# XuZhang1211/PVPUFormer

Measured on AMD Instinct MI355X. Metric: 448x448 images/sec fwd+bwd, ViT-B VPUFormer, higher is better.
Workload: dtype bf16

## Files before the change

include/vpu_hip.h:

```cpp
#ifndef VPU_HIP_H
#define VPU_HIP_H
#include <stdint.h>

#ifdef __cplusplus
extern "C" {
#endif

#define VPU_BF16 0
#define VPU_F32 1

#define VPU_EPI_BIAS 1
#define VPU_EPI_PREACT 2
#define VPU_EPI_GELU 4
#define VPU_EPI_RELU 8
#define VPU_EPI_DGELU 16
#define VPU_EPI_DRELU 32
#define VPU_EPI_RESID 64
#define VPU_EPI_AFFINE 128
#define VPU_EPI_ACCUM 256
#define VPU_EPI_OUT_F32 512
#define VPU_EPI_SAVE_DGELU 1024
#define VPU_EPI_MULAUX 2048

typedef struct vpu_gemm_desc {
// ... 171 lines not shown
                             void* stream);
int vpu_pixel_shuffle2_gn_stats(const void* in, void* out, const float* bias, double* stats, int32_t B, int32_t h, int32_t w,
                                int32_t C, int32_t dtype, void* stream);
int vpu_groupnorm_apply(const void* x, const float* w, const float* b, void* y, float* mean, float* rstd, const double* stats,
                        int32_t B, int64_t HW, int32_t C, float eps, int32_t gelu, int32_t dtype, void* stream);
int vpu_pixel_unshuffle2_nblk(int32_t C);
int vpu_pixel_unshuffle2_sums(const void* in, void* out, float* part, int32_t B, int32_t h, int32_t w, int32_t C,
                              int32_t dtype, void* stream);
int vpu_groupnorm_nchunk(void);
int vpu_groupnorm_fwd(const void* x, const float* w, const float* b, void* y, float* mean, float* rstd, double* stats,
                      int32_t B, int64_t HW, int32_t C, float eps, int32_t gelu, int32_t dtype, void* stream);
int vpu_groupnorm_bwd(const void* dy, const void* x, const float* w, const float* b, const float* mean,
                      const float* rstd, void* dx, float* part, double* stats, int32_t B, int64_t HW, int32_t C,
                      int32_t gelu, int32_t dtype, void* stream);
int vpu_bilinear_cl_fwd(const void* in, int32_t ld_in, void* out, int32_t ld_out, int32_t B, int32_t h, int32_t w,
                        int32_t H, int32_t W, int32_t C, int32_t dtype, void* stream);
int vpu_bilinear_cl_bwd(const void* dout, int32_t ld_out, void* din, int32_t ld_in, int32_t B, int32_t h, int32_t w,
                        int32_t H, int32_t W, int32_t C, int32_t dtype, void* stream);
int vpu_upsum_relu(void* io, const void* const* z, const int32_t* h, const int32_t* w, int32_t n, int32_t B, int32_t H,
                   int32_t W, int32_t C, int32_t dtype, void* stream);
int vpu_head_grad_fused(const void* dfn, const void* y, const float* inv, const float* dout, const void* x, const float* w,
                        const float* mask, void* dx, float* part, float* part_b, int64_t rows, int64_t HW, int32_t C,
                        int32_t dtype, void* stream);
int vpu_gate_stats(const void* Q, const void* Kt, float* cg, int32_t* argq, float* sg, int32_t* argc, int32_t B,
                   int32_t nq, int32_t N, int32_t C, int32_t dtype, void* stream);
int vpu_gate_apply(const void* x, const float* cg, const float* sg, void* out, int32_t B, int32_t N, int32_t C,
                   int32_t dtype, void* stream);
int vpu_gate_bwd(const void* dout, const void* x, const float* cg, const int32_t* argq, const float* sg,
                 const int32_t* argc, void* dx, int32_t accum, void* dQ, void* dK, float* part, int32_t B, int32_t nq,
                 int32_t N, int32_t C, int32_t dtype, void* stream);
int vpu_gate_fwd_n(const void* const* Q, const void* const* K, const void* x, void* const* out, float* cg, int32_t* argq,
                   float* sg, int32_t* argc, int32_t n, int32_t B, int32_t nq, int32_t N, int32_t C, int32_t dtype, void* stream);
int vpu_gate_bwd_n(const void* const* dout, const void* x, const float* cg, const int32_t* argq, const float* sg,
                   const int32_t* argc, void* dx, int32_t accum, void* const* dQ, void* const* dK, float* part, int32_t n,
                   int32_t B, int32_t nq, int32_t N, int32_t C, int32_t dtype, void* stream);
int vpu_convseg_fwd(const void* x, const float* w, const float* bias, const float* mask, float* out, int64_t rows,
                    int64_t HW, int32_t C, int32_t dtype, void* stream);
int vpu_convseg_bwd_nblk(int64_t rows);
int vpu_convseg_bwd(const float* dout, const void* x, const float* w, const float* mask, void* dx, int32_t accum,
                    float* part, float* part_b, int64_t rows, int64_t HW, int32_t C, int32_t dtype, void* stream);

int vpu_upsample_ac_fwd(const float* in, float* out, int64_t planes, int32_t h, int32_t w, int32_t H, int32_t W,
                        void* stream);
int vpu_upsample_ac_bwd(const float* dout, float* din, int64_t planes, int32_t h, int32_t w, int32_t H, int32_t W,
                        void* stream);
int vpu_p2cl_fwd_bwd(const float* prob, const float* gt, const int32_t* slot_mask_idx, const float* override_masks,
// ... 28 lines not shown
```

pvpuformer_amd/_lib.py:

```python
import ctypes as C
import os

_HERE = os.path.dirname(os.path.abspath(__file__))
LIB_PATH = os.path.join(_HERE, os.environ.get("VPU_LIB_FILE") or
                        ("libvpu_hip_diag.so" if os.environ.get("VPU_LIB_DIAG", "0") == "1" else "libvpu_hip.so"))

BF16, F32 = 0, 1

EPI_BIAS, EPI_PREACT, EPI_GELU, EPI_RELU, EPI_DGELU, EPI_DRELU = 1, 2, 4, 8, 16, 32
EPI_RESID, EPI_AFFINE, EPI_ACCUM, EPI_OUT_F32 = 64, 128, 256, 512
EPI_SAVE_DGELU, EPI_MULAUX = 1024, 2048


class GemmDesc(C.Structure):
    _fields_ = [
        ("A", C.c_void_p), ("B", C.c_void_p), ("C", C.c_void_p), ("bias", C.c_void_p), ("resid", C.c_void_p),
        ("aux", C.c_void_p), ("preact", C.c_void_p),
        ("M", C.c_int32), ("N", C.c_int32), ("K", C.c_int32),
        ("lda", C.c_int32), ("ldb", C.c_int32), ("ldc", C.c_int32), ("ldr", C.c_int32), ("ldaux", C.c_int32),
        ("batch", C.c_int32), ("inner", C.c_int32),
        ("sAo", C.c_int64), ("sAi", C.c_int64), ("sBo", C.c_int64), ("sBi", C.c_int64),
        ("sCo", C.c_int64), ("sCi", C.c_int64), ("sRo", C.c_int64), ("sRi", C.c_int64),
        ("transA", C.c_int32), ("transB", C.c_int32), ("dtype", C.c_int32), ("flags", C.c_int32),
        ("resid_period", C.c_int32),
# ... 74 lines not shown
    "vpu_masked_argmax": [_P, _P, _P, _I, _I, _I, _P],
    "vpu_error_masks": [_P, _P, _P, _P, _I, _I, _P],
    "vpu_roi_resize_batched": [_P, _I, _P, _I, _I, _I, _I, _P],
    "vpu_roi_paste_batched": [_P, _I, _P, _I, _I, _F, _F, _I, _P],
    "vpu_click_keys_batched": [_P, _I, _P, _P, _P, _I, _I, _I, _P],
    "vpu_box_prompts_batched": [_P, _I, _P, _I, _I, _I, _F, _P, _P, _P, _P, _P, _I, _P, _P, _P],
    "vpu_disk_maps": [_P, _P, _P, _I, _I, _I, _I, _F, _P],
    "vpu_patch_im2col": [_P, _P, _P, _I, _I, _I, _I, _I, _I, _P],
    "vpu_patch_im2col_prenorm": [_P, _P, _P, _I, _I, _I, _I, _I, _I, _P],
    "vpu_patch_im2col_floor": [_P, _P, _P, _I, _I, _I, _I, _I, _I, _I, _P],
    "vpu_window_permute": [_P, _P, _I, _I, _I, _I, _I, _I, _P],
    "vpu_space_to_depth2_crop": [_P, _P, _I, _I, _I, _I, _I, _P],
    "vpu_pixel_shuffle2": [_P, _P, _P, _I, _I, _I, _I, _I, _I, _P],
    "vpu_pixel_shuffle2_gn_stats": [_P, _P, _P, _P, _I, _I, _I, _I, _I, _P],
    "vpu_groupnorm_apply": [_P, _P, _P, _P, _P, _P, _P, _I, _L, _I, _F, _I, _I, _P],
    "vpu_pixel_unshuffle2_nblk": [_I],
    "vpu_pixel_unshuffle2_sums": [_P, _P, _P, _I, _I, _I, _I, _I, _P],
    "vpu_groupnorm_nchunk": [],
    "vpu_groupnorm_fwd": [_P, _P, _P, _P, _P, _P, _P, _I, _L, _I, _F, _I, _I, _P],
    "vpu_groupnorm_bwd": [_P, _P, _P, _P, _P, _P, _P, _P, _P, _I, _L, _I, _I, _I, _P],
    "vpu_bilinear_cl_fwd": [_P, _I, _P, _I, _I, _I, _I, _I, _I, _I, _I, _P],
    "vpu_bilinear_cl_bwd": [_P, _I, _P, _I, _I, _I, _I, _I, _I, _I, _I, _P],
    "vpu_head_grad_fused": [_P, _P, _P, _P, _P, _P, _P, _P, _P, _P, _L, _L, _I, _I, _P],
    "vpu_upsum_relu": [_P, C.POINTER(C.c_void_p), C.POINTER(C.c_int32), C.POINTER(C.c_int32), _I, _I, _I, _I, _I, _I, _P],
    "vpu_gate_stats": [_P, _P, _P, _P, _P, _P, _I, _I, _I, _I, _I, _P],
    "vpu_gate_apply": [_P, _P, _P, _P, _I, _I, _I, _I, _P],
    "vpu_gate_bwd": [_P, _P, _P, _P, _P, _P, _P, _I, _P, _P, _P, _I, _I, _I, _I, _I, _P],
    "vpu_gate_fwd_n": [C.POINTER(C.c_void_p), C.POINTER(C.c_void_p), _P, C.POINTER(C.c_void_p), _P, _P, _P, _P, _I, _I, _I, _I, _I, _I, _P],
    "vpu_gate_bwd_n": [C.POINTER(C.c_void_p), _P, _P, _P, _P, _P, _P, _I, C.POINTER(C.c_void_p), C.POINTER(C.c_void_p), _P, _I, _I, _I,
                       _I, _I, _I, _P],
    "vpu_convseg_fwd": [_P, _P, _P, _P, _P, _L, _L, _I, _I, _P],
    "vpu_convseg_bwd_nblk": [_L],
    "vpu_convseg_bwd": [_P, _P, _P, _P, _P, _I, _P, _P, _L, _L, _I, _I, _P],
    "vpu_upsample_ac_fwd": [_P, _P, _L, _I, _I, _I, _I, _P],
    "vpu_upsample_ac_bwd": [_P, _P, _L, _I, _I, _I, _I, _P],
    "vpu_p2cl_fwd_bwd": [_P, _P, _P, _P, _P, _P, _F, _I, _I, _I, _I, _P],
    "vpu_p2cl_up_nband": [_I, _I],
    "vpu_p2cl_up_fwd_bwd": [_P, _P, _P, _P, _P, _P, _F, _I, _I, _I, _I, _I, _I, _P],
    "vpu_nfl_dice_scratch_doubles": [_I],
    "vpu_nfl_dice_fwd_bwd": [_P, _P, _P, _P, _P, _F, _F, _I, _L, _P],
    "vpu_loss_finalize": [_P, _P, _I, _I, C.c_double, _F, _F, _F, _F, _P, _P],
    "vpu_adam_step": [_P, _P, _P, _P, _P, _L, _F, _F, _F, _F, _F, _I, _F, _P],
    "vpu_adam_step_groups": [_P, _P, _P, _P, _P, _L, _P, _P, _P, _I, _F, _F, _F, _I, _I, _F, _P],
    "vpu_adam_step_hyper": [_P, _P, _P, _P, _P, _L, _P, _P, _P, _P, _I, _F, _F, _F, _F, _I, _P],
    "vpu_gemm_set_option": [C.c_char_p, _I],
    "vpu_gemm_get_option": [C.c_char_p, C.POINTER(C.c_int32)],
# ... 40 lines not shown
```

pvpuformer_amd/csrc/spatial.hip:

```cpp
#include <stdlib.h>
#include "vpu_common.h"
#include "interp_ac.h"
#include "../../include/vpu_hip.h"

#define DISPATCH_T(dtype, ...)                                   \
    if ((dtype) == VPU_BF16) { using T = bf16_t; __VA_ARGS__ }   \
    else if ((dtype) == VPU_F32) { using T = float; __VA_ARGS__ } \
    else { vpu_set_error("bad dtype"); return VPU_ERR_ARG; }
#define ST reinterpret_cast<hipStream_t>(stream)

namespace {

__constant__ float c_mean[3] = {0.485f, 0.456f, 0.406f};
__constant__ float c_std[3] = {0.229f, 0.224f, 0.225f};

template <typename T, bool NORM = true, bool VEC = true>
__global__ __launch_bounds__(256) void patch_im2col_kernel(const float* __restrict__ img4,
                                                           const float* __restrict__ disks, T* __restrict__ cols,
                                                           int B, int H, int W, int P, int wg) {
    const int gw = W / P, gh = H / P;
    const int K3 = 3 * P * P, K3P = (K3 + 7) / 8 * 8;
    const int Tn = gw * gh, KK = 2 * K3P, chunks = KK / 8;
    const int64_t total = (int64_t)B * Tn * chunks;
    const int nwx = gw / wg;
// ... 1296 lines not shown
            for (int j = 0; j < 8; ++j) {
                dwa[j] += d * xv[j] * mk[j];
                const float t = iv * (g[j] - yv[j] * sdot) + d * wv[j] * mk[j];
                o[j] = xv[j] > 0.f ? t : 0.f;
            }
            store8(dx + row * C + c8, o);
        }
    }
#pragma unroll
    for (int j = 0; j < 8; ++j)
        for (int o = lpr; o < 64; o <<= 1) dwa[j] += __shfl_xor(dwa[j], o, 64);
    dba = wave_sum(dba);
    if (sub == 0) {
#pragma unroll
        for (int j = 0; j < 8; ++j) red[wave][c8 + j] = dwa[j];
    }
    if (lane == 0) redb[wave] = dba;
    __syncthreads();
    for (int c = threadIdx.x; c < C; c += 256)
        part[(int64_t)blockIdx.x * C + c] = red[0][c] + red[1][c] + red[2][c] + red[3][c];
    if (threadIdx.x == 0) part_b[blockIdx.x] = redb[0] + redb[1] + redb[2] + redb[3];
}

__global__ __launch_bounds__(256) void upsample_ac_fwd_kernel(const float* __restrict__ in, float* __restrict__ out,
                                                              int64_t planes, int h, int w, int H, int W) {
    const float sh = ac_scale(h, H), sw = ac_scale(w, W);
    const int64_t total = planes * H * W;
    for (int64_t i = (int64_t)blockIdx.x * 256 + threadIdx.x; i < total; i += (int64_t)gridDim.x * 256) {
        const int X = (int)(i % W), Y = (int)((i / W) % H);
        const int64_t pl = i / ((int64_t)W * H);
        out[i] = ac_sample(in + pl * h * w, w, h, w, sh, sw, Y, X);
    }
}
__global__ __launch_bounds__(256) void upsample_ac_bwd_kernel(const float* __restrict__ dout, float* __restrict__ din,
                                                              int64_t planes, int h, int w, int H, int W) {
    const float sh = H > 1 ? (float)(h - 1) / (float)(H - 1) : 0.f;
    const float sw = W > 1 ? (float)(w - 1) / (float)(W - 1) : 0.f;
    const float fh = sh > 0.f ? 1.f / sh : 0.f, fw = sw > 0.f ? 1.f / sw : 0.f;
    const int64_t total = planes * h * w;
    const bool small = total < ((int64_t)1 << 31);
    for (int64_t i = (int64_t)blockIdx.x * 256 + threadIdx.x; i < total; i += (int64_t)gridDim.x * 256) {
        int x, y;
        int64_t pl;
        if (small) {
            const unsigned iu = (unsigned)i, q = iu / (unsigned)w;
            x = (int)(iu - q * (unsigned)w); y = (int)(q % (unsigned)h); pl = q / (unsigned)h;
// ... 351 lines not shown
        return vpu_check_launch("vpu_convseg_bwd");
    }
    DISPATCH_T(dtype, convseg_bwd_kernel<T><<<nblk, 256, 0, ST>>>(dout, (const T*)x, w, mask, (T*)dx, accum, part,
                                                                 part_b, rows, HW, C, nblk);)
    return vpu_check_launch("vpu_convseg_bwd");
}
extern "C" int vpu_head_grad_fused(const void* dfn, const void* y, const float* inv, const float* dout, const void* x,
                                   const float* w, const float* mask, void* dx, float* part, float* part_b, int64_t rows,
                                   int64_t HW, int32_t C, int32_t dtype, void* stream) {
    vpu_clear_stale_error();
    if (dtype != VPU_BF16 || !(C == 64 || C == 128 || C == 256 || C == 512) || !dfn || !y || !inv || !dout || !x || !w ||
        !dx || !part || !part_b || rows < 1 ||
        (reinterpret_cast<uintptr_t>(dfn) | reinterpret_cast<uintptr_t>(y) | reinterpret_cast<uintptr_t>(x) |
         reinterpret_cast<uintptr_t>(dx)) % 16 != 0 ||
        (reinterpret_cast<uintptr_t>(w) | reinterpret_cast<uintptr_t>(mask)) % 32 != 0) {
        vpu_set_error("head_grad_fused: bf16, C in {64,128,256,512}, 16-byte aligned maps, 32-byte aligned w / mask");
        return VPU_ERR_ARG;
    }
    const int nblk = vpu_convseg_bwd_nblk(rows);
    head_grad_fused_kernel<<<nblk, 256, 0, ST>>>((const bf16_t*)dfn, (const bf16_t*)y, inv, dout, (const bf16_t*)x, w, mask,
                                                 (bf16_t*)dx, part, part_b, rows, HW, C, nblk);
    return vpu_check_launch("vpu_head_grad_fused");
}
extern "C" int vpu_upsample_ac_fwd(const float* in, float* out, int64_t planes, int32_t h, int32_t w, int32_t H,
                                   int32_t W, void* stream) {
    vpu_clear_stale_error();
    upsample_ac_fwd_kernel<<<vpu_grid_for(planes * H * W, 256, 65536), 256, 0, ST>>>(in, out, planes, h, w, H, W);
    return vpu_check_launch("vpu_upsample_ac_fwd");
}
extern "C" int vpu_upsample_ac_bwd(const float* dout, float* din, int64_t planes, int32_t h, int32_t w, int32_t H,
                                   int32_t W, void* stream) {
    vpu_clear_stale_error();
    upsample_ac_bwd_kernel<<<vpu_grid_for(planes * h * w, 256, 65536), 256, 0, ST>>>(dout, din, planes, h, w, H, W);
    return vpu_check_launch("vpu_upsample_ac_bwd");
}
```

pvpuformer_amd/engine.py:

```python
import contextlib
import math
import os
from collections import OrderedDict
from types import SimpleNamespace

import numpy as np
import torch

from . import ops
from ._lib import (BF16, F32, EPI_BIAS, EPI_PREACT, EPI_GELU, EPI_RELU, EPI_DGELU, EPI_DRELU, EPI_RESID, EPI_AFFINE,
                   EPI_ACCUM, EPI_OUT_F32, EPI_SAVE_DGELU, EPI_MULAUX)


class Tape:
    __slots__ = ("fns", "out_grads", "done", "sim_low", "lane")

    def __init__(self):
        self.fns = []
        self.out_grads = [None, None, None]
        self.done = False
        self.sim_low = None
        self.lane = None

    def append(self, fn):
# ... 89 lines not shown
        self.shadow_valid = False
        self._const_ready = False
        self.use_flash = True
        self.use_side = os.environ.get("VPU_WGRAD_STREAM", "0") == "1"
        self.side = None
        self.fuse_ln_pe = True
        self.group_wgrad = True
        self.ride_wgrad = True
        self.wgrad_fill = 0.8
        hid = self.D * c["mlp_ratio"]
        blk = sum(((n + 255) // 256) * ((k + 127) // 128) for n, k in ((3 * self.D, self.D), (self.D, self.D), (hid, self.D), (self.D, hid)))
        pk = os.environ.get("VPU_WGRAD_PACK", "")
        k3 = ops.gemm_get_option("k3")
        k4_default = (k3 & 8) != 0
        self.pack_wgrad = pk == "1" or (pk != "0" and (blk < 0.95 * 256 or k4_default))
        self.k3_wgrad = (k3 & 1) != 0
        self.k4_wgrad = (k3 & 8) != 0
        self.wgrad_round = 256 if (self.k4_wgrad or not self.k3_wgrad) else 512
        self.wgrad_tn = 256 if self.k4_wgrad else 128
        self.unify_wgrad = True
        self.lazy_zero = True
        self.xattn_split = max(1, int(os.environ.get("VPU_XATTN_SPLIT", "1")))
        self.neck_lanes = int(os.environ.get("VPU_NECK_LANES", "0"))
        self._tok_stream = None
        self._in_lanes = False
        self.dist_colsum = True
        self._pack_seen, self._pack_total = {}, {}
        self._pending_reports, self._reporting = [], False
        self.group_tiles = 256
        self.split_wgrad = True
        self._wq = []
        self._csq = []
        self._gq = []
        self._gq_out = set()
        self._frozen = set()
        self._token_rows = 0
        self.grad_ready_hook = None
        self.report_lag = max(1, int(os.environ.get("VPU_DIST_REPORT_LAG", "2")))

    def bind(self, named_params):
        self.names = OrderedDict()
        off = 0
        for n, p in named_params.items():
            self.names[n] = (off, tuple(p.shape), p.numel())
            off = _rup(off + p.numel(), 8)
        self.total = off
# ... 975 lines not shown
        if cx.training:
            def bwd_fusion():
                if fused.g is None:
                    return
                if relu_done[0]:
                    dt_ = fused.g
                else:
                    dt_ = self._new(B * HW4, Cc)
                    ops.act_bwd(fused.g, Cc, fused.t, Cc, dt_, Cc, B * HW4, Cc, 0, self.dt)
                self._wgrad(dt_, Cc, ys[0].t, Cc, gf, Cc, Cc, B * HW4, ldc=ldf, bias="head.fusion_conv.conv.bias")
                fuse_mask = self.dt == BF16
                mk = dict(flags=EPI_DRELU, ldaux=Cc) if fuse_mask else {}
                self._dgrad(dt_, Cc, wf, ldf, ys[0], B * HW4, Cc, Cc, **(dict(mk, aux=ys[0].t) if fuse_mask else {}))
                ymask[0][0] = fuse_mask
                for i in (1, 2, 3):
                    s = feats[i][1]
                    dz = self._new(B * s * s, Cc)
                    ops.bilinear_cl_bwd(dt_, Cc, dz, Cc, B, s, s, Hs, Hs, Cc, self.dt)
                    self._wgrad(dz, Cc, ys[i].t, Cc, (gf[0], gf[1] + i * Cc), Cc, Cc, B * s * s, ldc=ldf)
                    self._dgrad(dz, Cc, (wf[0], wf[1] + i * Cc), ldf, ys[i], B * s * s, Cc, Cc,
                                **(dict(mk, aux=ys[i].t) if fuse_mask else {}))
                    ymask[i][0] = fuse_mask
            self.tape.append(bwd_fusion)
        seg = self._new(B * HW4, dtype=torch.float32)
        ops.convseg_fwd(fused.t, self.Pm("head.conv_seg.weight"), self.Pm("head.conv_seg.bias"), drop_mask, seg,
                        B * HW4, HW4, Cc)
        dm = self.cfg["head_d_model"]
        query = self.mlp(q_out, "head.ffn_layer.lin1", "head.ffn_layer.lin2", B * nq, dm, 2 * dm, Cc, "relu")
        qn, fn = Var(torch.empty_like(query.t)), Var(torch.empty_like(fused.t))
        inv_q, inv_f = self._new(B * nq, dtype=torch.float32), self._new(B * HW4, dtype=torch.float32)
        ops.l2norm_fwd(query.t, qn.t, inv_q, B * nq, Cc)
        ops.l2norm_fwd(fused.t, fn.t, inv_f, B * HW4, Cc)
        sim = self._new(B, nq, HW4, dtype=torch.float32)
        ops.gemm(qn.t, fn.t, sim, nq, HW4, Cc, Cc, Cc, HW4, self.dt, flags=EPI_OUT_F32 | EPI_AFFINE, post_mul=0.5,
                 post_add=0.5, batch=B, inner=1, sA=(nq * Cc, 0), sB=(HW4 * Cc, 0), sC=(nq * HW4, 0))
        if cx.taps is not None:
            cx.taps["seg_lowres"] = seg.view(B, 1, Hs, Hs)
            cx.taps["sim_lowres"] = sim.view(B, nq, Hs, Hs)
            cx.taps["fused"] = fused.t
        inst = self._new(B, 1, H, W_, dtype=torch.float32)
        ops.upsample_ac_fwd(seg, inst, B, Hs, Hs, H, W_)
        aux = None
        self.sim_low = sim.view(B, nq, Hs, Hs)
        if materialize_aux:
            aux = self._new(B, nq, H, W_, dtype=torch.float32)
            ops.upsample_ac_fwd(sim, aux, B * nq, Hs, Hs, H, W_)
        tape.sim_low = self.sim_low
        if cx.training:
            def bwd_head():
                d_inst, d_aux, d_sim_low = tape.out_grads
                if d_aux is not None or d_sim_low is not None:
                    if d_sim_low is not None:
                        dsim = d_sim_low.view(B, nq, HW4)
                    else:
                        dsim = self._new(B, nq, HW4, dtype=torch.float32)
                        ops.upsample_ac_bwd(d_aux, dsim, B * nq, Hs, Hs, H, W_)
                    if self.dt == BF16:
                        dsim_t = self._new(B, nq, HW4)
                        ops.cast2d(dsim, HW4, dsim_t, HW4, B * nq, HW4)
                    else:
                        dsim_t = dsim
                    qn.g, fn.g = torch.empty_like(qn.t), torch.empty_like(fn.t)
                    ops.gemm(dsim_t, fn.t, qn.g, nq, Cc, HW4, HW4, Cc, Cc, self.dt, transB=True, alpha=0.5, batch=B,
                             inner=1, sA=(nq * HW4, 0), sB=(HW4 * Cc, 0), sC=(nq * Cc, 0))
                    ops.gemm(dsim_t, qn.t, fn.g, HW4, Cc, nq, HW4, Cc, Cc, self.dt, transA=True, transB=True, alpha=0.5,
                             batch=B, inner=1, sA=(nq * HW4, 0), sB=(nq * Cc, 0), sC=(HW4 * Cc, 0))
                    query.g = torch.empty_like(query.t)
                    ops.l2norm_bwd(qn.g, qn.t, inv_q, query.g, B * nq, Cc)
                    one_pass = d_inst is not None and self.dt == BF16 and Cc in (64, 128, 256, 512)
                    if not one_pass:
                        fused.g = torch.empty_like(fused.t)
                        ops.l2norm_bwd(fn.g, fn.t, inv_f, fused.g, B * HW4, Cc)
                if d_inst is not None:
# ... 306 lines not shown
```

pvpuformer_amd/ops.py:

```python
import ctypes as C

import torch

from . import _lib
from ._lib import (BF16, F32, EPI_BIAS, EPI_PREACT, EPI_GELU, EPI_RELU, EPI_DGELU, EPI_DRELU, EPI_RESID, EPI_AFFINE,
                   EPI_ACCUM, EPI_OUT_F32, EPI_SAVE_DGELU, EPI_MULAUX, GemmDesc)

TORCH_DTYPE = {BF16: torch.bfloat16, F32: torch.float32}


def code_of(t):
    if isinstance(t, tuple):
        t = t[0]
    if t.dtype == torch.bfloat16:
        return BF16
    if t.dtype == torch.float32:
        return F32
    raise TypeError(f"unsupported dtype {t.dtype}")


_raw_stream = getattr(torch._C, "_cuda_getCurrentRawStream", None)
_cur_device = getattr(torch._C, "_cuda_getDevice", None)


# ... 492 lines not shown
def gate_bwd_n(douts, x, cg, argq, sg, argc, dx, accum, dQs, dKs, part, B, nq, N, Cdim):
    _lib.call("vpu_gate_bwd_n", _ptr_array(douts), ptr(x), ptr(cg), ptr(argq), ptr(sg), ptr(argc), ptr(dx), int(accum),
              _ptr_array(dQs), _ptr_array(dKs), ptr(part), len(douts), B, nq, N, Cdim, code_of(x), _stream())


def convseg_fwd(x, w, bias, mask, out, rows, HW, Cdim):
    _lib.call("vpu_convseg_fwd", ptr(x), ptr(w), ptr(bias), ptr(mask), ptr(out), rows, HW, Cdim, code_of(x), _stream())


def convseg_bwd_nblk(rows):
    return _lib.load().vpu_convseg_bwd_nblk(rows)


def convseg_bwd(dout, x, w, mask, dx, accum, part, part_b, rows, HW, Cdim):
    _lib.call("vpu_convseg_bwd", ptr(dout), ptr(x), ptr(w), ptr(mask), ptr(dx), int(accum), ptr(part), ptr(part_b),
              rows, HW, Cdim, code_of(x), _stream())


def head_grad_fused(dfn, y, inv, dout, x, w, mask, dx, part, part_b, rows, HW, Cdim):
    _lib.call("vpu_head_grad_fused", ptr(dfn), ptr(y), ptr(inv), ptr(dout), ptr(x), ptr(w), ptr(mask), ptr(dx), ptr(part),
              ptr(part_b), rows, HW, Cdim, code_of(x), _stream())


def upsample_ac_fwd(inp, out, planes, h, w, H, W):
    _lib.call("vpu_upsample_ac_fwd", ptr(inp), ptr(out), planes, h, w, H, W, _stream())


def upsample_ac_bwd(dout, din, planes, h, w, H, W):
    _lib.call("vpu_upsample_ac_bwd", ptr(dout), ptr(din), planes, h, w, H, W, _stream())


def p2cl_fwd_bwd(prob, gt, slot_idx, override, loss_part, dprob, grad_scale, B, S, H, W):
    _lib.call("vpu_p2cl_fwd_bwd", ptr(prob), ptr(gt), ptr(slot_idx), ptr(override), ptr(loss_part), ptr(dprob),
              grad_scale, B, S, H, W, _stream())


def p2cl_up_fwd_bwd(sim_low, gt, slot_idx, override, loss_part, dsim_low, grad_scale, B, S, h, w, H, W):
    nband = _lib.load().vpu_p2cl_up_nband(h, w)
    bands = torch.empty(B * S, nband, device=sim_low.device, dtype=torch.float32)
    _lib.call("vpu_p2cl_up_fwd_bwd", ptr(sim_low), ptr(gt), ptr(slot_idx), ptr(override), ptr(bands), ptr(dsim_low),
              grad_scale, B, S, h, w, H, W, _stream())
    if loss_part is None:
        return bands
    torch.sum(bands, dim=1, out=loss_part.view(B * S))
    return loss_part

# ... 27 lines not shown
```

Before: 998.8.

## Fuse head conv_seg, feature L2 norm and similarity GEMM into row kernels

Adds fused forward and backward kernels for the segmentation head. The forward kernel computes the per-pixel inverse norm, the conv_seg dot product and the query-feature similarity with MFMA in a single pass over the fused features, so the normalized feature map is never written out. The backward kernel computes dx, including the L2-norm backward, conv_seg grad and ReLU mask, together with per-block partial query gradients. Separate small kernels reduce the query-gradient partials and the weight sums. This removes several full passes over the large feature map and a separate GEMM launch, at the cost of considerable new kernel complexity, and it applies only to bf16 with restricted C and nq.

```diff
diff --git a/include/vpu_hip.h b/include/vpu_hip.h
--- a/include/vpu_hip.h
+++ b/include/vpu_hip.h
@@ -217,6 +217,13 @@
 int vpu_head_grad_fused(const void* dfn, const void* y, const float* inv, const float* dout, const void* x, const float* w,
                         const float* mask, void* dx, float* part, float* part_b, int64_t rows, int64_t HW, int32_t C,
                         int32_t dtype, void* stream);
+int vpu_head_rows_fwd(const void* x, const void* qn, const float* w, const float* bias, const float* mask, float* seg,
+                      float* inv, float* sim, int32_t B, int64_t HW, int32_t nq, int32_t C, int32_t dtype, void* stream);
+int vpu_head_rows_bwd_nblk(int32_t B, int64_t HW, int32_t C);
+int vpu_head_rows_bwd(const void* x, const float* inv, const void* qn, const float* inv_q, const float* dsim,
+                      const float* dseg, const float* w, const float* mask, void* dx, float* part, float* part_b,
+                      float* dqn_part, void* dquery, int32_t B, int64_t HW, int32_t nq, int32_t C, int32_t dtype,
+                      void* stream);
 int vpu_gate_stats(const void* Q, const void* Kt, float* cg, int32_t* argq, float* sg, int32_t* argc, int32_t B,
                    int32_t nq, int32_t N, int32_t C, int32_t dtype, void* stream);
 int vpu_gate_apply(const void* x, const float* cg, const float* sg, void* out, int32_t B, int32_t N, int32_t C,
diff --git a/pvpuformer_amd/_lib.py b/pvpuformer_amd/_lib.py
--- a/pvpuformer_amd/_lib.py
+++ b/pvpuformer_amd/_lib.py
@@ -120,6 +120,9 @@
     "vpu_bilinear_cl_fwd": [_P, _I, _P, _I, _I, _I, _I, _I, _I, _I, _I, _P],
     "vpu_bilinear_cl_bwd": [_P, _I, _P, _I, _I, _I, _I, _I, _I, _I, _I, _P],
     "vpu_head_grad_fused": [_P, _P, _P, _P, _P, _P, _P, _P, _P, _P, _L, _L, _I, _I, _P],
+    "vpu_head_rows_fwd": [_P, _P, _P, _P, _P, _P, _P, _P, _I, _L, _I, _I, _I, _P],
+    "vpu_head_rows_bwd_nblk": [_I, _L, _I],
+    "vpu_head_rows_bwd": [_P, _P, _P, _P, _P, _P, _P, _P, _P, _P, _P, _P, _P, _I, _L, _I, _I, _I, _P],
     "vpu_upsum_relu": [_P, C.POINTER(C.c_void_p), C.POINTER(C.c_int32), C.POINTER(C.c_int32), _I, _I, _I, _I, _I, _I, _P],
     "vpu_gate_stats": [_P, _P, _P, _P, _P, _P, _I, _I, _I, _I, _I, _P],
     "vpu_gate_apply": [_P, _P, _P, _P, _I, _I, _I, _I, _P],
diff --git a/pvpuformer_amd/csrc/spatial.hip b/pvpuformer_amd/csrc/spatial.hip
--- a/pvpuformer_amd/csrc/spatial.hip
+++ b/pvpuformer_amd/csrc/spatial.hip
@@ -1342,6 +1342,363 @@
     if (threadIdx.x == 0) part_b[blockIdx.x] = redb[0] + redb[1] + redb[2] + redb[3];
 }
 
+typedef __bf16 bf16x4_t __attribute__((ext_vector_type(4)));
+__device__ __forceinline__ void hr_unpack(const uint4& u, float (&v)[8]) {
+    const bf16x8_t e = __builtin_bit_cast(bf16x8_t, u);
+#pragma unroll
+    for (int j = 0; j < 8; ++j) v[j] = (float)e[j];
+}
+__device__ __forceinline__ bf16x8_t hr_frag(const char* img, int row, int ld, int k) {
+    return *reinterpret_cast<const bf16x8_t*>(img + row * ld + k * 2);
+}
+constexpr int HR_LDP = 64 * 2 + 16;
+
+template <int C>
+__global__ __launch_bounds__(256) void head_rows_fwd_kernel(const bf16_t* __restrict__ x, const bf16_t* __restrict__ qn,
+                                                            const float* __restrict__ w, const float* __restrict__ bias,
+                                                            const float* __restrict__ mask, float* __restrict__ seg,
+                                                            float* __restrict__ inv, float* __restrict__ sim, int HW, int nq,
+                                                            int ntiles) {
+    extern __shared__ __attribute__((aligned(16))) char hr_lds[];
+    constexpr int LPR = C / 8, RPW = 64 / LPR, TRIPS = 16 / RPW, LD = C * 2 + 16;
+    char* sQ = hr_lds;
+    char* sF = sQ + nq * LD;
+    float* sS = reinterpret_cast<float*>(sF + 64 * LD);
+    const int tid = threadIdx.x, lane = tid & 63, wave = tid >> 6, sub = lane / LPR, cl = lane - sub * LPR;
+    const int b = blockIdx.y;
+    for (int i = tid; i < nq * LPR; i += 256) {
+        const int q = i / LPR, c8 = (i - q * LPR) * 8;
+        *reinterpret_cast<uint4*>(sQ + q * LD + c8 * 2) = *reinterpret_cast<const uint4*>(qn + ((int64_t)b * nq + q) * C + c8);
+    }
+    float ww[8], wm[8];
+    load8(w + cl * 8, ww);
+    if (mask) {
+        float mk[8];
+        load8(mask + (int64_t)b * C + cl * 8, mk);
+#pragma unroll
+        for (int j = 0; j < 8; ++j) wm[j] = ww[j] * mk[j];
+    } else {
+#pragma unroll
+        for (int j = 0; j < 8; ++j) wm[j] = ww[j];
+    }
+    const float b0 = bias[0];
+    const bf16_t* xb = x + (int64_t)b * HW * C;
+    const int prow = wave * 16 + sub;
+    uint4 raw[TRIPS];
+    int tile = blockIdx.x;
+    if (tile < ntiles) {
+#pragma unroll
+        for (int t = 0; t < TRIPS; ++t) {
+            const int hw = tile * 64 + prow + t * RPW;
+            raw[t] = make_uint4(0, 0, 0, 0);
+            if (hw < HW) raw[t] = *reinterpret_cast<const uint4*>(xb + (int64_t)hw * C + cl * 8);
+        }
+    }
+    for (; tile < ntiles; tile += gridDim.x) {
+        const int hw0 = tile * 64;
+#pragma unroll
+        for (int t = 0; t < TRIPS; ++t) {
+            const int p = prow + t * RPW, hw = hw0 + p;
+            float v[8];
+            hr_unpack(raw[t], v);
+            float s = 0.f, sg = 0.f;
+#pragma unroll
+            for (int j = 0; j < 8; ++j) s += v[j] * v[j];
+#pragma unroll
+            for (int j = 0; j < 8; ++j) sg += v[j] * wm[j];
+            for (int o = LPR >> 1; o > 0; o >>= 1) s += __shfl_xor(s, o, 64);
+            for (int o = LPR >> 1; o > 0; o >>= 1) sg += __shfl_xor(sg, o, 64);
+            const float iv = 1.0f / fmaxf(sqrtf(s), 1e-12f);
+            if (cl == 0 && hw < HW) {
+                inv[(int64_t)b * HW + hw] = iv;
+                seg[(int64_t)b * HW + hw] = sg + b0;
+            }
+            bf16x8_t f;
+#pragma unroll
+            for (int j = 0; j < 8; ++j) f[j] = (bf16_t)(v[j] * iv);
+            *reinterpret_cast<bf16x8_t*>(sF + p * LD + cl * 16) = f;
+        }
+        const int next = tile + gridDim.x;
+        if (next < ntiles) {
+#pragma unroll
+            for (int t = 0; t < TRIPS; ++t) {
+                const int hw = next * 64 + prow + t * RPW;
+                raw[t] = make_uint4(0, 0, 0, 0);
+                if (hw < HW) raw[t] = *reinterpret_cast<const uint4*>(xb + (int64_t)hw * C + cl * 8);
+            }
+        }
+        __syncthreads();
+        bf16x8_t fb[C / 32];
+#pragma unroll
+        for (int ks = 0; ks < C / 32; ++ks) fb[ks] = hr_frag(sF, wave * 16 + (lane & 15), LD, ks * 32 + 8 * (lane >> 4));
+        for (int mt = 0; mt < (nq >> 4); ++mt) {
+            f32x4_t acc = (f32x4_t){0.f, 0.f, 0.f, 0.f};
+#pragma unroll
+            for (int ks = 0; ks < C / 32; ++ks)
+                acc = __builtin_amdgcn_mfma_f32_16x16x32_bf16(hr_frag(sQ, mt * 16 + (lane & 15), LD, ks * 32 + 8 * (lane >> 4)),
+                                                              fb[ks], acc, 0, 0, 0);
+#pragma unroll
+            for (int r = 0; r < 4; ++r) sS[(mt * 16 + 4 * (lane >> 4) + r) * 64 + wave * 16 + (lane & 15)] = acc[r] * 0.5f + 0.5f;
+        }
+        __syncthreads();
+        if (hw0 + lane < HW)
+            for (int q = wave; q < nq; q += 4) sim[((int64_t)b * nq + q) * HW + hw0 + lane] = sS[q * 64 + lane];
+    }
+}
+
+template <int C>
+__global__ __launch_bounds__(256) void head_rows_bwd_kernel(const bf16_t* __restrict__ x, const float* __restrict__ inv,
+                                                            const bf16_t* __restrict__ qn, const float* __restrict__ dsim,
+                                                            const float* __restrict__ dseg, const float* __restrict__ w,
+                                                            const float* __restrict__ mask, bf16_t* __restrict__ dx,
+                                                            float* __restrict__ dqp, int HW, int nq, int ntiles_all, int G, int tpc) {
+    extern __shared__ __attribute__((aligned(16))) char hr_lds[];
+    constexpr int LPR = C / 8, RPW = 64 / LPR, TRIPS = 16 / RPW, LD = C * 2 + 16, NCT = C / 64;
+    const int KQ = (nq + 31) & ~31, LDQ = KQ * 2 + 16, nqt = nq >> 4, nks = KQ >> 5;
+    char* sQT = hr_lds;
+    char* sDT = sQT + C * LDQ;
+    char* sD = sDT + 64 * LDQ;
+    char* sGY = sD + 64 * HR_LDP;
+    const int tid = threadIdx.x, lane = tid & 63, wave = tid >> 6, sub = lane / LPR, cl = lane - sub * LPR, c8 = cl * 8;
+    const int b = blockIdx.x / G, g0 = blockIdx.x - b * G;
+    for (int i = tid; i < C * LDQ / 16; i += 256) reinterpret_cast<uint4*>(sQT)[i] = make_uint4(0, 0, 0, 0);
+    __syncthreads();
+    for (int i = tid; i < nq * LPR; i += 256) {
+        const int q = i / LPR, cc = (i - q * LPR) * 8;
+        const bf16x8_t e = *reinterpret_cast<const bf16x8_t*>(qn + ((int64_t)b * nq + q) * C + cc);
+#pragma unroll
+        for (int j = 0; j < 8; ++j) *reinterpret_cast<bf16_t*>(sQT + (cc + j) * LDQ + q * 2) = e[j];
+    }
+    float wv[8], mk[8] = {1.f, 1.f, 1.f, 1.f, 1.f, 1.f, 1.f, 1.f};
+    load8(w + c8, wv);
+    if (mask) load8(mask + (int64_t)b * C + c8, mk);
+    f32x4_t dq[4][NCT];
+#pragma unroll
+    for (int mt = 0; mt < 4; ++mt)
+#pragma unroll
+        for (int ct = 0; ct < NCT; ++ct) dq[mt][ct] = (f32x4_t){0.f, 0.f, 0.f, 0.f};
+    const int64_t rowb = (int64_t)b * HW;
+    const bf16_t* xb = x + rowb * C;
+    const float* dsb = dsim + (int64_t)b * nq * HW;
+    const int prow = wave * 16 + sub;
+    const int sp = tid & 63, sqg = tid >> 6;
+    constexpr bool PF = C <= 256;
+    uint4 raw[TRIPS], nraw[PF ? TRIPS : 1];
+    float ivr[TRIPS], dr[TRIPS], nivr[PF ? TRIPS : 1], ndr[PF ? TRIPS : 1], dsv[2][8], ndsv[2][8];
+#define HR_ISSUE(TILE_, RAW_, IV_, D_, DS_)                                                                            \
+    {                                                                                                                  \
+        _Pragma("unroll") for (int t = 0; t < TRIPS; ++t) {                                                            \
+            const int hw = (TILE_) * 64 + prow + t * RPW;                                                              \
+            RAW_[t] = make_uint4(0, 0, 0, 0);                                                                          \
+            IV_[t] = 0.f;                                                                                              \
+            D_[t] = 0.f;                                                                                               \
+            if (hw < HW) {                                                                                             \
+                RAW_[t] = *reinterpret_cast<const uint4*>(xb + (int64_t)hw * C + c8);                                  \
+                IV_[t] = inv[rowb + hw];                                                                               \
+                D_[t] = dseg[rowb + hw];                                                                               \
+            }                                                                                                          \
+        }                                                                                                              \
+        _Pragma("unroll") for (int u = 0; u < 2; ++u) _Pragma("unroll") for (int j = 0; j < 8; ++j) {                  \
+            const int q = (sqg + 4 * u) * 8 + j, hw = (TILE_) * 64 + sp;                                               \
+            DS_[u][j] = (q < nq && hw < HW) ? dsb[(int64_t)q * HW + hw] : 0.f;                                         \
+        }                                                                                                              \
+    }
+    int tile = g0 * tpc;
+    const int ntiles = (g0 + 1) * tpc < ntiles_all ? (g0 + 1) * tpc : ntiles_all;
+    if (tile < ntiles) HR_ISSUE(tile, raw, ivr, dr, dsv)
+    for (; tile < ntiles; ++tile) {
+        const int hw0 = tile * 64;
+#pragma unroll
+        for (int u = 0; u < 2; ++u) {
+            const int qg = sqg + 4 * u;
+            if (qg * 8 < KQ) {
+                bf16x8_t e;
+#pragma unroll
+                for (int j = 0; j < 8; ++j) e[j] = (bf16_t)dsv[u][j];
+                *reinterpret_cast<bf16x8_t*>(sDT + sp * LDQ + qg * 16) = e;
+                if (qg * 8 < nq) {
+#pragma unroll
+                    for (int j = 0; j < 8; ++j) *reinterpret_cast<bf16_t*>(sD + (qg * 8 + j) * HR_LDP + sp * 2) = e[j];
+                }
+            }
+        }
+#pragma unroll
+        for (int t = 0; t < TRIPS; ++t) {
+            float v[8];
+            hr_unpack(raw[t], v);
+            bf16x8_t f;
+#pragma unroll
+            for (int j = 0; j < 8; ++j) f[j] = (bf16_t)(v[j] * ivr[t]);
+            *reinterpret_cast<bf16x8_t*>(sGY + (prow + t * RPW) * LD + cl * 16) = f;
+        }
+        __syncthreads();
+        const int next = tile + 1;
+        if constexpr (PF) { if (next < ntiles) HR_ISSUE(next, nraw, nivr, ndr, ndsv) }
+#pragma unroll 1
+        for (int ks = 0; ks < 2; ++ks) {
+            bf16x8_t fa[4];
+#pragma unroll
+            for (int mt = 0; mt < 4; ++mt)
+                if (mt < nqt) fa[mt] = hr_frag(sD, mt * 16 + (lane & 15), HR_LDP, ks * 32 + 8 * (lane >> 4));
+#pragma unroll
+            for (int ct = 0; ct < NCT; ++ct) {
+                const int c = wave * (C / 4) + ct * 16 + (lane & 15);
+                bf16x8_t fb;
+#pragma unroll
+                for (int j = 0; j < 8; ++j)
+                    fb[j] = *reinterpret_cast<const bf16_t*>(sGY + (ks * 32 + 8 * (lane >> 4) + j) * LD + c * 2);
+#pragma unroll
+                for (int mt = 0; mt < 4; ++mt)
+                    if (mt < nqt) dq[mt][ct] = __builtin_amdgcn_mfma_f32_16x16x32_bf16(fa[mt], fb, dq[mt][ct], 0, 0, 0);
+            }
+        }
+        __syncthreads();
+        {
+            bf16x8_t fd[2];
+#pragma unroll
+            for (int ks = 0; ks < 2; ++ks)
+                if (ks < nks) fd[ks] = hr_frag(sDT, wave * 16 + (lane & 15), LDQ, ks * 32 + 8 * (lane >> 4));
+#pragma unroll 2
+            for (int ct = 0; ct < C / 16; ++ct) {
+                f32x4_t acc = (f32x4_t){0.f, 0.f, 0.f, 0.f};
+#pragma unroll
+                for (int ks = 0; ks < 2; ++ks)
+                    if (ks < nks)
+                        acc = __builtin_amdgcn_mfma_f32_16x16x32_bf16(
+                            hr_frag(sQT, ct * 16 + (lane & 15), LDQ, ks * 32 + 8 * (lane >> 4)), fd[ks], acc, 0, 0, 0);
+                bf16x4_t e;
+#pragma unroll
+                for (int r = 0; r < 4; ++r) e[r] = (bf16_t)(acc[r] * 0.5f);
+                *reinterpret_cast<bf16x4_t*>(sGY + (wave * 16 + (lane & 15)) * LD + (ct * 16 + 4 * (lane >> 4)) * 2) = e;
+            }
+        }
+        __syncthreads();
+#pragma unroll
+        for (int t = 0; t < TRIPS; ++t) {
+            const int p = prow + t * RPW, hw = hw0 + p;
+            const bool live = hw < HW;
+            float xv[8], gv[8], yv[8];
+            hr_unpack(raw[t], xv);
+            hr_unpack(*reinterpret_cast<const uint4*>(sGY + p * LD + cl * 16), gv);
+            const float iv = ivr[t], d = dr[t];
+#pragma unroll
+            for (int j = 0; j < 8; ++j) yv[j] = (float)(bf16_t)(xv[j] * iv);
+            float sdot = 0.f;
+#pragma unroll
+            for (int j = 0; j < 8; ++j) sdot += gv[j] * yv[j];
+            for (int o = LPR >> 1; o > 0; o >>= 1) sdot += __shfl_xor(sdot, o, 64);
+            if (live) {
+                float o[8];
+#pragma unroll
+                for (int j = 0; j < 8; ++j) {
+                    const float tt = iv * (gv[j] - yv[j] * sdot) + d * wv[j] * mk[j];
+                    o[j] = xv[j] > 0.f ? tt : 0.f;
+                }
+                store8(dx + (rowb + hw) * C + c8, o);
+            }
+        }
+        __syncthreads();
+        if constexpr (PF) {
+            if (next < ntiles) {
+#pragma unroll
+                for (int t = 0; t < TRIPS; ++t) { raw[t] = nraw[t]; ivr[t] = nivr[t]; dr[t] = ndr[t]; }
+#pragma unroll
+                for (int u = 0; u < 2; ++u)
+#pragma unroll
+                    for (int j = 0; j < 8; ++j) dsv[u][j] = ndsv[u][j];
+            }
+        } else {
+            if (next < ntiles) HR_ISSUE(next, raw, ivr, dr, dsv)
+        }
+    }
+#undef HR_ISSUE
+    float* dqo = dqp + (int64_t)blockIdx.x * nq * C;
+#pragma unroll
+    for (int mt = 0; mt < 4; ++mt)
+        if (mt < nqt) {
+#pragma unroll
+            for (int ct = 0; ct < NCT; ++ct)
+#pragma unroll
+                for (int r = 0; r < 4; ++r)
+                    dqo[(mt * 16 + 4 * (lane >> 4) + r) * C + wave * (C / 4) + ct * 16 + (lane & 15)] = dq[mt][ct][r];
+        }
+}
+
+__global__ __launch_bounds__(256) void head_rows_wsum_kernel(const float* __restrict__ dout, const bf16_t* __restrict__ x,
+                                                             const float* __restrict__ mask, float* __restrict__ part,
+                                                             float* __restrict__ part_b, int64_t rows, int64_t HW, int C,
+                                                             int nblk) {
+    __shared__ float red[4][512];
+    __shared__ float redb[4];
+    const int lane = threadIdx.x & 63, wave = threadIdx.x >> 6;
+    const int lpr = C >> 3, rpp = 64 / lpr;
+    const int sub = lane / lpr, c8 = (lane % lpr) * 8;
+    float dwa[8] = {0.f, 0.f, 0.f, 0.f, 0.f, 0.f, 0.f, 0.f};
+    float dba = 0.f;
+    const int64_t per = (rows + nblk - 1) / nblk;
+    const int64_t r0 = (int64_t)blockIdx.x * per, r1 = r0 + per < rows ? r0 + per : rows;
+    float mk[8] = {1.f, 1.f, 1.f, 1.f, 1.f, 1.f, 1.f, 1.f};
+    int64_t mk_b = -1;
+    int64_t bimg = (r0 + (int64_t)wave * rpp + sub) / HW, brem = (r0 + (int64_t)wave * rpp + sub) - bimg * HW;
+    for (int64_t rb = r0 + (int64_t)wave * rpp; rb < r1; rb += 4 * rpp, brem += 4 * rpp) {
+        const int64_t row = rb + sub;
+        while (brem >= HW) { brem -= HW; ++bimg; }
+        if (row < r1) {
+            float xv[8];
+            load8(x + row * C + c8, xv);
+            const float d = dout[row];
+            if (c8 == 0) dba += d;
+            if (mask && bimg != mk_b) { load8(mask + bimg * C + c8, mk); mk_b = bimg; }
+#pragma unroll
+            for (int j = 0; j < 8; ++j) dwa[j] += d * xv[j] * mk[j];
+        }
+    }
+#pragma unroll
+    for (int j = 0; j < 8; ++j)
+        for (int o = lpr; o < 64; o <<= 1) dwa[j] += __shfl_xor(dwa[j], o, 64);
+    dba = wave_sum(dba);
+    if (sub == 0) {
+#pragma unroll
+        for (int j = 0; j < 8; ++j) red[wave][c8 + j] = dwa[j];
+    }
+    if (lane == 0) redb[wave] = dba;
+    __syncthreads();
+    for (int c = threadIdx.x; c < C; c += 256)
+        part[(int64_t)blockIdx.x * C + c] = red[0][c] + red[1][c] + red[2][c] + red[3][c];
+    if (threadIdx.x == 0) part_b[blockIdx.x] = redb[0] + redb[1] + redb[2] + redb[3];
+}
+
+__global__ __launch_bounds__(256) void head_rows_qgrad_kernel(const float* __restrict__ dqp, const bf16_t* __restrict__ qn,
+                                                              const float* __restrict__ inv_q, bf16_t* __restrict__ dquery,
+                                                              int rows, int nq, int G, int C) {
+    const int lpr = C >> 3, rpw = 64 / lpr;
+    const int lane = threadIdx.x & 63, sub = lane / lpr, cl = lane - sub * lpr;
+    const int row = (blockIdx.x * 4 + (threadIdx.x >> 6)) * rpw + sub;
+    float d[8] = {0.f, 0.f, 0.f, 0.f, 0.f, 0.f, 0.f, 0.f}, yv[8] = {0.f, 0.f, 0.f, 0.f, 0.f, 0.f, 0.f, 0.f};
+    if (row < rows) {
+        const int b = row / nq, q = row - b * nq;
+        for (int g = 0; g < G; ++g) {
+            float t[8];
+            load8(dqp + (((int64_t)b * G + g) * nq + q) * C + cl * 8, t);
+#pragma unroll
+            for (int j = 0; j < 8; ++j) d[j] += t[j];
+        }
+#pragma unroll
+        for (int j = 0; j < 8; ++j) d[j] = (float)(bf16_t)(d[j] * 0.5f);
+        load8(qn + (int64_t)row * C + cl * 8, yv);
+    }
+    float s = 0.f;
+#pragma unroll
+    for (int j = 0; j < 8; ++j) s += d[j] * yv[j];
+    for (int o = lpr >> 1; o > 0; o >>= 1) s += __shfl_xor(s, o, 64);
+    if (row < rows) {
+        const float iv = inv_q[row];
+#pragma unroll
+        for (int j = 0; j < 8; ++j) d[j] = iv * (d[j] - yv[j] * s);
+        store8(dquery + (int64_t)row * C + cl * 8, d);
+    }
+}
+
 __global__ __launch_bounds__(256) void upsample_ac_fwd_kernel(const float* __restrict__ in, float* __restrict__ out,
                                                               int64_t planes, int h, int w, int H, int W) {
     const float sh = ac_scale(h, H), sw = ac_scale(w, W);
@@ -1739,6 +2096,99 @@
                                                  (bf16_t*)dx, part, part_b, rows, HW, C, nblk);
     return vpu_check_launch("vpu_head_grad_fused");
 }
+static bool head_rows_shape_ok(int32_t B, int64_t HW, int32_t nq, int32_t C, int32_t dtype) {
+    return dtype == VPU_BF16 && (C == 64 || C == 128 || C == 256 || C == 512) && nq >= 16 && nq <= 64 && nq % 16 == 0 && B >= 1 &&
+           B <= 65535 && HW >= 1 && HW < (1 << 24);
+}
+static size_t head_rows_fwd_lds(int nq, int C) { return (size_t)(nq + 64) * (C * 2 + 16) + (size_t)nq * 64 * 4; }
+static size_t head_rows_bwd_lds(int nq, int C) {
+    const int KQ = (nq + 31) & ~31;
+    return (size_t)(C + 64) * (KQ * 2 + 16) + 64 * HR_LDP + (size_t)64 * (C * 2 + 16);
+}
+extern "C" int vpu_head_rows_fwd(const void* x, const void* qn, const float* w, const float* bias, const float* mask,
+                                 float* seg, float* inv, float* sim, int32_t B, int64_t HW, int32_t nq, int32_t C,
+                                 int32_t dtype, void* stream) {
+    vpu_clear_stale_error();
+    if (!head_rows_shape_ok(B, HW, nq, C, dtype) || !x || !qn || !w || !bias || !seg || !inv || !sim ||
+        (reinterpret_cast<uintptr_t>(x) | reinterpret_cast<uintptr_t>(qn)) % 16 != 0 ||
+        (reinterpret_cast<uintptr_t>(w) | reinterpret_cast<uintptr_t>(mask)) % 32 != 0) {
+        vpu_set_error("head_rows_fwd: bf16, C in {64,128,256,512}, nq in {16,32,48,64}, 16-byte aligned x / qn, 32-byte aligned w / mask");
+        return VPU_ERR_ARG;
+    }
+    const int ntiles = (int)((HW + 63) / 64);
+    int G = 512 / B;
+    G = G < 1 ? 1 : (G > ntiles ? ntiles : G);
+    const size_t lds = head_rows_fwd_lds(nq, C);
+#define VPU_HR_FWD(C_)                                                                                                  \
+    case C_: {                                                                                                          \
+        static VpuDevOnce attr;                                                                                         \
+        if (auto todo_ = attr.pending()) { VPU_SET_LDS((int)head_rows_fwd_lds(64, C_), head_rows_fwd_kernel<C_>); }      \
+        head_rows_fwd_kernel<C_><<<dim3(G, B), 256, lds, ST>>>((const bf16_t*)x, (const bf16_t*)qn, w, bias, mask, seg, inv, \
+                                                              sim, (int)HW, nq, ntiles);                                \
+    } break;
+    switch (C) { VPU_HR_FWD(64) VPU_HR_FWD(128) VPU_HR_FWD(256) VPU_HR_FWD(512) }
+#undef VPU_HR_FWD
+    return vpu_check_launch("vpu_head_rows_fwd");
+}
+static void head_rows_slices(int32_t B, int64_t HW, int32_t C, int* G, int* tpc) {
+    const int64_t K = HW, BK = 64, tiles = (int64_t)((C + 127) / 128) * B;
+    int64_t kchunk = (K + BK - 1) / BK * BK, splitk = 1;
+    if ((tiles < 192 || (tiles <= 256 && K >= 32 * BK)) && K >= 8 * BK) {
+        int64_t want = (384 + tiles - 1) / tiles;
+        if (want > K / (4 * BK)) want = K / (4 * BK);
+        if (want > 128) want = 128;
+        if (want > 1) {
+            kchunk = ((K + want - 1) / want + BK - 1) / BK * BK;
+            splitk = (K + kchunk - 1) / kchunk;
+        }
+    }
+    *G = (int)splitk;
+    *tpc = (int)(kchunk / BK);
+}
+extern "C" int vpu_head_rows_bwd_nblk(int32_t B, int64_t HW, int32_t C) {
+    vpu_clear_stale_error();
+    if (B < 1 || HW < 1 || C < 1) return 1;
+    int G, tpc;
+    head_rows_slices(B, HW, C, &G, &tpc);
+    return B * G;
+}
+extern "C" int vpu_head_rows_bwd(const void* x, const float* inv, const void* qn, const float* inv_q, const float* dsim,
+                                 const float* dseg, const float* w, const float* mask, void* dx, float* part, float* part_b,
+                                 float* dqn_part, void* dquery, int32_t B, int64_t HW, int32_t nq, int32_t C, int32_t dtype,
+                                 void* stream) {
+    vpu_clear_stale_error();
+    if (!head_rows_shape_ok(B, HW, nq, C, dtype) || !x || !inv || !qn || !inv_q || !dsim || !dseg || !w || !dx || !part ||
+        !part_b || !dqn_part || !dquery ||
+        (reinterpret_cast<uintptr_t>(x) | reinterpret_cast<uintptr_t>(qn) | reinterpret_cast<uintptr_t>(dx) |
+         reinterpret_cast<uintptr_t>(dquery)) % 16 != 0 ||
+        (reinterpret_cast<uintptr_t>(w) | reinterpret_cast<uintptr_t>(mask) | reinterpret_cast<uintptr_t>(dqn_part)) % 32 != 0) {
+        vpu_set_error("head_rows_bwd: bf16, C in {64,128,256,512}, nq in {16,32,48,64}, 16-byte aligned maps, 32-byte aligned w / mask / partials");
+        return VPU_ERR_ARG;
+    }
+    const int ntiles = (int)((HW + 63) / 64);
+    int G, tpc;
+    head_rows_slices(B, HW, C, &G, &tpc);
+    const int nblk = B * G;
+    const size_t lds = head_rows_bwd_lds(nq, C);
+#define VPU_HR_BWD(C_)                                                                                                  \
+    case C_: {                                                                                                          \
+        static VpuDevOnce attr;                                                                                         \
+        if (auto todo_ = attr.pending()) { VPU_SET_LDS((int)head_rows_bwd_lds(64, C_), head_rows_bwd_kernel<C_>); }      \
+        head_rows_bwd_kernel<C_><<<nblk, 256, lds, ST>>>((const bf16_t*)x, inv, (const bf16_t*)qn, dsim, dseg, w, mask,  \
+                                                        (bf16_t*)dx, dqn_part, (int)HW, nq, ntiles, G, tpc);            \
+    } break;
+    switch (C) { VPU_HR_BWD(64) VPU_HR_BWD(128) VPU_HR_BWD(256) VPU_HR_BWD(512) }
+#undef VPU_HR_BWD
+    if (int rc = vpu_check_launch("vpu_head_rows_bwd")) return rc;
+    const int rows = B * nq, rpb = 4 * (64 / (C >> 3));
+    head_rows_qgrad_kernel<<<(rows + rpb - 1) / rpb, 256, 0, ST>>>(dqn_part, (const bf16_t*)qn, inv_q, (bf16_t*)dquery, rows, nq,
+                                                                  G, C);
+    if (int rc = vpu_check_launch("vpu_head_rows_bwd")) return rc;
+    const int64_t nrows = (int64_t)B * HW;
+    const int nb = vpu_convseg_bwd_nblk(nrows);
+    head_rows_wsum_kernel<<<nb, 256, 0, ST>>>(dseg, (const bf16_t*)x, mask, part, part_b, nrows, HW, C, nb);
+    return vpu_check_launch("vpu_head_rows_bwd");
+}
 extern "C" int vpu_upsample_ac_fwd(const float* in, float* out, int64_t planes, int32_t h, int32_t w, int32_t H,
                                    int32_t W, void* stream) {
     vpu_clear_stale_error();
diff --git a/pvpuformer_amd/engine.py b/pvpuformer_amd/engine.py
--- a/pvpuformer_amd/engine.py
+++ b/pvpuformer_amd/engine.py
@@ -135,6 +135,7 @@
         self.lazy_zero = True
         self.xattn_split = max(1, int(os.environ.get("VPU_XATTN_SPLIT", "1")))
         self.neck_lanes = int(os.environ.get("VPU_NECK_LANES", "0"))
+        self.head_rows = os.environ.get("VPU_HEAD_ROWS", "1") != "0"
         self._tok_stream = None
         self._in_lanes = False
         self.dist_colsum = True
@@ -1156,18 +1157,24 @@
                                 **(dict(mk, aux=ys[i].t) if fuse_mask else {}))
                     ymask[i][0] = fuse_mask
             self.tape.append(bwd_fusion)
+        rows = self.head_rows and not materialize_aux and ops.head_rows_ok(self.dt, Cc, nq)
         seg = self._new(B * HW4, dtype=torch.float32)
-        ops.convseg_fwd(fused.t, self.Pm("head.conv_seg.weight"), self.Pm("head.conv_seg.bias"), drop_mask, seg,
-                        B * HW4, HW4, Cc)
+        if not rows:
+            ops.convseg_fwd(fused.t, self.Pm("head.conv_seg.weight"), self.Pm("head.conv_seg.bias"), drop_mask, seg,
+                            B * HW4, HW4, Cc)
         dm = self.cfg["head_d_model"]
         query = self.mlp(q_out, "head.ffn_layer.lin1", "head.ffn_layer.lin2", B * nq, dm, 2 * dm, Cc, "relu")
-        qn, fn = Var(torch.empty_like(query.t)), Var(torch.empty_like(fused.t))
+        qn, fn = Var(torch.empty_like(query.t)), Var(None if rows else torch.empty_like(fused.t))
         inv_q, inv_f = self._new(B * nq, dtype=torch.float32), self._new(B * HW4, dtype=torch.float32)
         ops.l2norm_fwd(query.t, qn.t, inv_q, B * nq, Cc)
-        ops.l2norm_fwd(fused.t, fn.t, inv_f, B * HW4, Cc)
         sim = self._new(B, nq, HW4, dtype=torch.float32)
-        ops.gemm(qn.t, fn.t, sim, nq, HW4, Cc, Cc, Cc, HW4, self.dt, flags=EPI_OUT_F32 | EPI_AFFINE, post_mul=0.5,
-                 post_add=0.5, batch=B, inner=1, sA=(nq * Cc, 0), sB=(HW4 * Cc, 0), sC=(nq * HW4, 0))
+        if rows:
+            ops.head_rows_fwd(fused.t, qn.t, self.Pm("head.conv_seg.weight"), self.Pm("head.conv_seg.bias"), drop_mask, seg,
+                              inv_f, sim, B, HW4, nq, Cc)
+        else:
+            ops.l2norm_fwd(fused.t, fn.t, inv_f, B * HW4, Cc)
+            ops.gemm(qn.t, fn.t, sim, nq, HW4, Cc, Cc, Cc, HW4, self.dt, flags=EPI_OUT_F32 | EPI_AFFINE, post_mul=0.5,
+                     post_add=0.5, batch=B, inner=1, sA=(nq * Cc, 0), sB=(HW4 * Cc, 0), sC=(nq * HW4, 0))
         if cx.taps is not None:
             cx.taps["seg_lowres"] = seg.view(B, 1, Hs, Hs)
             cx.taps["sim_lowres"] = sim.view(B, nq, Hs, Hs)
@@ -1183,6 +1190,27 @@
         if cx.training:
             def bwd_head():
                 d_inst, d_aux, d_sim_low = tape.out_grads
+                if rows and d_inst is not None and (d_aux is not None or d_sim_low is not None):
+                    if d_sim_low is not None:
+                        dsim = d_sim_low.view(B, nq, HW4)
+                    else:
+                        dsim = self._new(B, nq, HW4, dtype=torch.float32)
+                        ops.upsample_ac_bwd(d_aux, dsim, B * nq, Hs, Hs, H, W_)
+                    dseg = self._new(B * HW4, dtype=torch.float32)
+                    ops.upsample_ac_bwd(d_inst, dseg, B, Hs, Hs, H, W_)
+                    nb = ops.convseg_bwd_nblk(B * HW4)
+                    part, part_b = self._new(nb, Cc, dtype=torch.float32), self._new(nb, dtype=torch.float32)
+                    dqn_part = self._new(ops.head_rows_bwd_nblk(B, HW4, Cc), nq, Cc, dtype=torch.float32)
+                    query.g, fused.g = torch.empty_like(query.t), torch.empty_like(fused.t)
+                    ops.head_rows_bwd(fused.t, inv_f, qn.t, inv_q, dsim, dseg, self.Pm("head.conv_seg.weight"), drop_mask,
+                                      fused.g, part, part_b, dqn_part, query.g, B, HW4, nq, Cc)
+                    relu_done[0] = True
+                    self._csq.append((part, self.G("head.conv_seg.weight"), nb, Cc))
+                    self._csq.append((part_b, self.G("head.conv_seg.bias"), nb, 1))
+                    return
+                if fn.t is None and (d_aux is not None or d_sim_low is not None):
+                    fn.t = torch.empty_like(fused.t)
+                    ops.l2norm_fwd(fused.t, fn.t, inv_f, B * HW4, Cc)
                 if d_aux is not None or d_sim_low is not None:
                     if d_sim_low is not None:
                         dsim = d_sim_low.view(B, nq, HW4)
diff --git a/pvpuformer_amd/ops.py b/pvpuformer_amd/ops.py
--- a/pvpuformer_amd/ops.py
+++ b/pvpuformer_amd/ops.py
@@ -538,6 +538,24 @@
               ptr(part_b), rows, HW, Cdim, code_of(x), _stream())
 
 
+def head_rows_ok(dtype_code, Cdim, nq):
+    return dtype_code == _lib.BF16 and Cdim in (64, 128, 256, 512) and nq % 16 == 0 and 16 <= nq <= 64
+
+
+def head_rows_fwd(x, qn, w, bias, mask, seg, inv, sim, B, HW, nq, Cdim):
+    _lib.call("vpu_head_rows_fwd", ptr(x), ptr(qn), ptr(w), ptr(bias), ptr(mask), ptr(seg), ptr(inv), ptr(sim), B, HW, nq,
+              Cdim, code_of(x), _stream())
+
+
+def head_rows_bwd_nblk(B, HW, Cdim):
+    return _lib.load().vpu_head_rows_bwd_nblk(B, HW, Cdim)
+
+
+def head_rows_bwd(x, inv, qn, inv_q, dsim, dseg, w, mask, dx, part, part_b, dqn_part, dquery, B, HW, nq, Cdim):
+    _lib.call("vpu_head_rows_bwd", ptr(x), ptr(inv), ptr(qn), ptr(inv_q), ptr(dsim), ptr(dseg), ptr(w), ptr(mask), ptr(dx),
+              ptr(part), ptr(part_b), ptr(dqn_part), ptr(dquery), B, HW, nq, Cdim, code_of(x), _stream())
+
+
 def upsample_ac_fwd(inp, out, planes, h, w, H, W):
     _lib.call("vpu_upsample_ac_fwd", ptr(inp), ptr(out), planes, h, w, H, W, _stream())
 
```

Measured after the change: 1003 (median of 6 runs). About the same (+0.5%).
